# Kamino666/video_features

Measured on AMD Instinct MI355X. Metric: frames/sec CLIP-ViT-B/32 uni_12, higher is better.
Workload: dtype bf16; 1 GPU; model=CLIP-ViT-B/32, global_batch=256, seq_len=12, resolution=224, parallelism=dp1

## Files before the change

### video_features_amd/models/clip_vit.py

```python
from __future__ import annotations

from dataclasses import dataclass
from typing import Optional

import torch
import torch.nn.functional as F
from torch import nn

from .. import ops


@dataclass
class ViTConfig:
    input_resolution: int = 224
    patch_size: int = 32
    width: int = 768
    layers: int = 12
    heads: int = 12
    output_dim: int = 512


VIT_B32 = ViTConfig(patch_size=32)
VIT_B16 = ViTConfig(patch_size=16)


class LayerNorm(nn.LayerNorm):
    def forward(self, x: torch.Tensor) -> torch.Tensor:
        return ops.layer_norm(x, self.weight, self.bias, self.eps)


class MultiheadSelfAttention(nn.Module):
    def __init__(self, width: int, heads: int):
        super().__init__()
        self.heads = heads
        self.head_dim = width // heads
        self.qkv = nn.Linear(width, 3 * width)
        self.proj = nn.Linear(width, width)

    def forward(self, x: torch.Tensor) -> torch.Tensor:
        o = ops.mhsa_fused(self.qkv(x), self.heads)
        return self.proj(o)


class MLP(nn.Module):
    def __init__(self, width: int):
        super().__init__()
        self.c_fc = nn.Linear(width, 4 * width)
        self.c_proj = nn.Linear(4 * width, width)

    def forward(self, x: torch.Tensor) -> torch.Tensor:
        h = ops.linear_act(x, self.c_fc.weight, self.c_fc.bias, 'quick_gelu')
        return self.c_proj(h)


class ResidualAttentionBlock(nn.Module):
    def __init__(self, width: int, heads: int):
        super().__init__()
        self.ln_1 = LayerNorm(width)
        self.attn = MultiheadSelfAttention(width, heads)
        self.ln_2 = LayerNorm(width)
        self.mlp = MLP(width)

    def forward(self, x: torch.Tensor) -> torch.Tensor:
        x = x + self.attn(self.ln_1(x))
        x = x + self.mlp(self.ln_2(x))
        return x


class VisionTransformer(nn.Module):
    def __init__(self, cfg: ViTConfig = VIT_B32):
        super().__init__()
        self.cfg = cfg
        w = cfg.width
        self.conv1 = nn.Conv2d(3, w, kernel_size=cfg.patch_size,
                               stride=cfg.patch_size, bias=False)
        n_patches = (cfg.input_resolution // cfg.patch_size) ** 2
        scale = w ** -0.5
        self.class_embedding = nn.Parameter(scale * torch.randn(w))
        self.positional_embedding = nn.Parameter(
            scale * torch.randn(n_patches + 1, w))
        self.ln_pre = LayerNorm(w)
        self.blocks = nn.ModuleList(
            [ResidualAttentionBlock(w, cfg.heads) for _ in range(cfg.layers)])
        self.ln_post = LayerNorm(w)
        self.proj = nn.Parameter(scale * torch.randn(w, cfg.output_dim))

    def _patch_embed(self, x: torch.Tensor) -> torch.Tensor:
        if x.is_cuda:
            t = x.shape[0]
            p = self.cfg.patch_size
            g = x.shape[-1] // p
            xp = x.reshape(t, 3, g, p, g, p).permute(0, 2, 4, 1, 3, 5)
            xp = xp.reshape(t, g * g, 3 * p * p)
            w = self.conv1.weight.reshape(self.cfg.width, -1)
            return xp @ w.t()
        x = self.conv1(x)
        return x.flatten(2).transpose(1, 2)

    def forward(self, x: torch.Tensor) -> torch.Tensor:
        x = self._patch_embed(x)
        x = ops.clip_embed_ln(x, self.class_embedding,
                              self.positional_embedding, self.ln_pre.weight,
                              self.ln_pre.bias, self.ln_pre.eps)
        full_tail = ops._env_flag('VFA_CLIP_FULL_TAIL')
        delta, res = None, x
        for blk in (self.blocks if full_tail else self.blocks[:-1]):
            if delta is None:
                y1, s1 = blk.ln_1(res), res
            else:
                y1, s1 = ops.layer_norm_residual(delta, res, blk.ln_1.weight,
                                                 blk.ln_1.bias, blk.ln_1.eps)
            a = blk.attn(y1)
            y2, s2 = ops.layer_norm_residual(a, s1, blk.ln_2.weight,
                                             blk.ln_2.bias, blk.ln_2.eps)
            delta, res = blk.mlp(y2), s2
        if full_tail:
            x = delta + res
            x = self.ln_post(x[:, 0, :])
        else:
            x = self._cls_tail(self.blocks[-1], delta, res)
        return x @ self.proj.to(x.dtype)

    def _cls_tail(self, blk: ResidualAttentionBlock,
                  delta: Optional[torch.Tensor],
                  res: torch.Tensor) -> torch.Tensor:
        w = self.cfg.width
        if delta is None:
            y1, s1 = blk.ln_1(res), res
        else:
            y1, s1 = ops.layer_norm_residual(delta, res, blk.ln_1.weight,
                                             blk.ln_1.bias, blk.ln_1.eps)
        qkv = blk.attn.qkv
        kv = F.linear(y1, qkv.weight[w:], qkv.bias[w:])
        q = F.linear(y1[:, 0], qkv.weight[:w], qkv.bias[:w])
        o = ops.attention_pool(q, kv, blk.attn.heads)
        a = blk.attn.proj(o)
        y2, s2 = ops.layer_norm_residual(a, s1[:, 0], blk.ln_2.weight,
                                         blk.ln_2.bias, blk.ln_2.eps)
        d = blk.mlp(y2)
        y, _ = ops.layer_norm_residual(d, s2, self.ln_post.weight,
                                       self.ln_post.bias, self.ln_post.eps)
        return y

    def encode_image(self, x: torch.Tensor) -> torch.Tensor:
        return self.forward(x)


def build_clip_vit(feature_type: str) -> VisionTransformer:
    if feature_type in ('CLIP-ViT-B/32', 'CLIP4CLIP-ViT-B-32'):
        return VisionTransformer(VIT_B32)
    if feature_type == 'CLIP-ViT-B/16':
        return VisionTransformer(VIT_B16)
    raise ValueError(f'unknown CLIP feature type {feature_type!r}')
```

### video_features_amd/ops/__init__.py

```python
from __future__ import annotations

import math
import os
from typing import Optional

import torch

_ext = None
_ext_err: Optional[str] = None


def _env_flag(name: str) -> bool:
    return os.environ.get(name, '').strip().lower() not in (
        '', '0', 'false', 'no', 'off')


def _load_extension():
    global _ext, _ext_err
    if _ext is not None or _ext_err is not None:
        return _ext
    try:
        from . import _vfa_hip
        _ext = _vfa_hip
    except ImportError as e:
# ... 345 lines not shown
            and kv.dtype == torch.bfloat16 and d == 64 and c == heads * 64):
        return _ext.attention_pool(q.contiguous(), kv.contiguous(),
                                   int(heads))
    qh = q.float().view(b, heads, 1, d)
    kh = kv[..., :c].float().reshape(b, l, heads, d).permute(0, 2, 1, 3)
    vh = kv[..., c:].float().reshape(b, l, heads, d).permute(0, 2, 1, 3)
    attn = (qh @ kh.transpose(-2, -1)) / math.sqrt(d)
    o = attn.softmax(dim=-1) @ vh
    return o.reshape(b, c).to(q.dtype)


_ACT_IDS = {'none': 0, 'relu': 1, 'quick_gelu': 2, 'gelu': 3,
            'leaky_relu': 4}


def _act_id(act: str) -> int:
    if act not in _ACT_IDS:
        raise ValueError(f'unknown activation {act!r}; expected one of '
                         f'{sorted(_ACT_IDS)}')
    return _ACT_IDS[act]


def _apply_act(y: torch.Tensor, act: str) -> torch.Tensor:
    _act_id(act)
    if act == 'relu':
        return torch.nn.functional.relu(y)
    if act == 'quick_gelu':
        return y * torch.sigmoid(1.702 * y)
    if act == 'gelu':
        return torch.nn.functional.gelu(y, approximate='tanh')
    if act == 'leaky_relu':
        return torch.nn.functional.leaky_relu(y, 0.1)
    return y


def linear_act(x: torch.Tensor, weight: torch.Tensor,
               bias: Optional[torch.Tensor] = None,
               act: str = 'none',
               res: Optional[torch.Tensor] = None) -> torch.Tensor:
    k = x.shape[-1]
    n = weight.shape[0]
    if (_use_hip(x) and x.dtype == torch.bfloat16
            and weight.dtype == torch.bfloat16 and k % 8 == 0 and n >= 16
            and not _env_flag('VFA_NO_LTGEMM')):
        x2 = x.reshape(-1, k).contiguous()
        r2 = res.reshape(-1, n).contiguous() if res is not None else None
        out = _ext.linear_act(x2, weight.contiguous(), bias, r2,
                              _act_id(act))
        return out.reshape(*x.shape[:-1], n)
    y = torch.nn.functional.linear(x, weight, bias)
    if res is not None:
        y = y + res.reshape(y.shape)
    return _apply_act(y, act)


def temporal_merge_fused(y: torch.Tensor, b: int, kt: int, st: int,
                         p0: int, relu: bool = False,
                         p1: Optional[int] = None) -> Optional[torch.Tensor]:
    if (_use_hip(y)
            and y.is_contiguous(memory_format=torch.channels_last)):
        return _ext.temporal_merge(y, b, kt, st, p0,
                                   p0 if p1 is None else p1, relu)
    return None


def conv1x1_act(x: torch.Tensor, weight: torch.Tensor,
                bias: Optional[torch.Tensor] = None, act: str = 'none',
                res: Optional[torch.Tensor] = None) -> torch.Tensor:
    b, cin, h, w = x.shape
    x2 = x.permute(0, 2, 3, 1).reshape(-1, cin)
    r2 = res.permute(0, 2, 3, 1).reshape(-1, weight.shape[0]) \
        if res is not None else None
    y = linear_act(x2, weight.reshape(weight.shape[0], cin), bias, act, r2)
    return y.reshape(b, h, w, weight.shape[0]).permute(0, 3, 1, 2)


def conv2d_act(x: torch.Tensor, weight: torch.Tensor,
               bias: Optional[torch.Tensor] = None,
               stride=1, padding=0, act: str = 'none',
               res: Optional[torch.Tensor] = None,
               out: Optional[torch.Tensor] = None,
               out_off: int = 0, dilation=1, in_off: int = 0,
               in_ch: Optional[int] = None) -> torch.Tensor:
    sh, sw = (stride, stride) if isinstance(stride, int) else stride
    dh, dw = (dilation, dilation) if isinstance(dilation, int) else dilation
    if in_ch is None:
        if in_off:
            raise ValueError('conv2d_act: in_off needs in_ch')
        cx = x.shape[1]
    else:
        cx = in_ch
    if isinstance(padding, int):
        pt = pb = pl = pr = padding
    elif len(padding) == 2:
        pt = pb = padding[0]
        pl = pr = padding[1]
    else:
        pt, pb, pl, pr = padding
    if (_use_hip(x) and x.dtype == torch.bfloat16
            and weight.dtype == torch.bfloat16
            and weight.shape[1] == (cx + 7) // 8 * 8
            and (in_ch is None or (in_ch % 8 == 0 and in_off % 8 == 0
                                   and x.shape[1] % 8 == 0))
            and x.is_contiguous(memory_format=torch.channels_last)
            and not _env_flag('VFA_NO_CONV')):
        if (weight.shape[2] == 1 and weight.shape[3] == 1
# ... 247 lines not shown
```

### video_features_amd/ops/csrc/bindings.cpp

```cpp
#include <torch/extension.h>
#include <c10/hip/HIPStream.h>
#include <mutex>
#include <unordered_map>
#include <hip/hip_runtime.h>
#include <hip/hip_bf16.h>

extern "C" {
void vfa_quick_gelu(const void*, void*, long long, int, hipStream_t);
void vfa_gelu_tanh(const void*, void*, long long, int, hipStream_t);
void vfa_layer_norm(const void*, const void*, const void*, void*, long long,
                    int, float, int, hipStream_t);
void vfa_bilinear_warp(const void*, const void*, void*, int, int, int, int,
                       int, hipStream_t);
void vfa_bilinear_warp_nhwc(const void*, const void*, void*, int, int, int,
                            int, long long, long long, long long, long long,
                            float, hipStream_t);
void vfa_pwc_correlation_nhwc(const void*, const void*, void*, int, int, int,
                              int, int, int, hipStream_t);
long long vfa_tconv_lds_bytes(int, int);
void vfa_tconv_pform(const void*, const void*, const void*, void*, void*, int,
                     int, int, int, int, int, int, hipStream_t);
void vfa_tconv_direct(const void*, const void*, const void*, void*, int, int,
                      int, int, long long, long long, long long, long long,
                      int, int, hipStream_t);
void vfa_grid_sample(const void*, const void*, void*, long long, int, int,
                     int, int, int, int, hipStream_t);
void vfa_corr_repack(const void*, void*, int, int, int, int, int,
                     hipStream_t);
void vfa_pwc_correlation(const void*, const void*, const void*, void*, int,
                         int, int, int, int, int, int, hipStream_t);
void vfa_mhsa_small(const void*, const void*, const void*, void*, int, int,
                    int, float, int, hipStream_t);
void vfa_flash_qkv(const void*, void*, int, int, int, float, hipStream_t);
void vfa_mfma_gemm16(const void*, const void*, void*, hipStream_t);
void vfa_layer_norm_residual(const void*, const void*, const void*,
                             const void*, void*, void*, long long, int,
                             float, int, hipStream_t);
void vfa_u8_chw_norm(const void*, void*, long long, int, int, const float*,
                     const float*, int, hipStream_t);
void vfa_corr_lookup(const void*, const void*, const void*, const void*,
                     const void*, void*, int, int, int, int, int, int, int,
                     int, int, long long, int, int, int, int, hipStream_t);
void vfa_convex_upsample(const void*, const void*, void*, int, int, int, int,
                         int, hipStream_t);
void vfa_gru_zr(const void*, const void*, void*, void*, int, int, int,
                long long, int, int, hipStream_t);
void vfa_gru_out(const void*, const void*, void*, int, int, int, long long,
                 int, int, hipStream_t);
void vfa_instance_norm2d(const void*, void*, int, int, int, float, int, int,
                         int, hipStream_t);
void vfa_maxpool3d_same(const void*, void*, long long, int, int, int, int,
                        int, int, int, int, int, int, int, int, int, int,
                        int, int, hipStream_t);
void vfa_maxpool2d_same(const void*, void*, long long, int, int, int, int,
                        int, int, int, int, int, int, int, int, int,
                        hipStream_t);
void vfa_linear_act(const void*, const void*, const void*, const void*,
                    void*, int, int, int, int, hipStream_t);
void vfa_temporal_merge(const void*, void*, int, int, int, int, int, int,
                        int, long long, int, int, hipStream_t);
void vfa_conv2d_nhwc(const void*, const void*, const void*, const void*,
                     const void*, void*, int, int, int, int, int, int, int,
                     int, int, int, int, int, int, int, int, int, int, int,
                     hipStream_t);
void vfa_conv2d_pick_tile(int, int, int*, int*);
void vfa_pad2d_nhwc(const void*, void*, int, int, int, int, int, int, int,
                    int, int, hipStream_t);
void vfa_avgpool2d_nhwc(const void*, void*, long long, int, int, int, int,
                        int, int, hipStream_t);
void vfa_attnpool_tokens(const void*, const void*, void*, long long, int, int,
                         hipStream_t);
void vfa_attention_pool_d64(const void*, const void*, void*, long long, int,
                            int, float, hipStream_t);
void vfa_clip_embed_ln(const void*, const void*, const void*, const void*,
                       const void*, void*, long long, int, int, float, int,
                       hipStream_t);
}

namespace {

int dtype_tag(const torch::Tensor& t) {
  switch (t.scalar_type()) {
    case torch::kFloat32: return 0;
    case torch::kBFloat16: return 1;
    case torch::kFloat16: return 2;
    default:
      TORCH_CHECK(false, "unsupported dtype ", t.scalar_type());
  }
}

hipStream_t current_stream() {
  return c10::hip::getCurrentHIPStream().stream();
}

torch::Tensor quick_gelu(torch::Tensor x) {
  TORCH_CHECK(x.is_cuda() && x.is_contiguous());
  auto out = torch::empty_like(x);
  vfa_quick_gelu(x.data_ptr(), out.data_ptr(), x.numel(), dtype_tag(x),
                 current_stream());
  return out;
}

torch::Tensor gelu_tanh(torch::Tensor x) {
  TORCH_CHECK(x.is_cuda() && x.is_contiguous());
  auto out = torch::empty_like(x);
  vfa_gelu_tanh(x.data_ptr(), out.data_ptr(), x.numel(), dtype_tag(x),
                current_stream());
  return out;
}
// ... 368 lines not shown
                             std::vector<int64_t> out_sz, bool nhwc) {
  TORCH_CHECK(x.is_cuda() && x.dim() == 4);
  if (nhwc) {
    TORCH_CHECK(cl_contig(x), "channels_last expected");
  } else {
    TORCH_CHECK(x.is_contiguous());
  }
  auto out = nhwc
      ? torch::empty({x.size(0), out_sz[0], out_sz[1], x.size(1)},
                     x.options()).permute({0, 3, 1, 2})
      : torch::empty({x.size(0), x.size(1), out_sz[0], out_sz[1]},
                     x.options());
  vfa_maxpool2d_same(x.data_ptr(), out.data_ptr(), x.size(0),
                     (int)x.size(1), (int)x.size(2), (int)x.size(3),
                     (int)out_sz[0], (int)out_sz[1], (int)kernel[0],
                     (int)kernel[1], (int)stride[0], (int)stride[1],
                     (int)pad_front[0], (int)pad_front[1], nhwc ? 1 : 0,
                     dtype_tag(x), current_stream());
  return out;
}

torch::Tensor linear_act(torch::Tensor x, torch::Tensor w,
                         c10::optional<torch::Tensor> bias,
                         c10::optional<torch::Tensor> res, int64_t act) {
  TORCH_CHECK(x.is_cuda() && x.dim() == 2 && x.is_contiguous());
  TORCH_CHECK(w.dim() == 2 && w.is_contiguous());
  TORCH_CHECK(x.scalar_type() == torch::kBFloat16 &&
              w.scalar_type() == torch::kBFloat16);
  const int m = (int)x.size(0), kk = (int)x.size(1), n = (int)w.size(0);
  TORCH_CHECK(w.size(1) == kk && kk % 8 == 0, "K%8==0 required");
  TORCH_CHECK(act >= 0 && act <= 4, "linear_act: unknown activation id ",
              act);
  const void* bptr = nullptr;
  torch::Tensor bc;
  if (bias.has_value()) {
    bc = bias->contiguous().to(torch::kBFloat16);
    TORCH_CHECK(bc.numel() == n);
    bptr = bc.data_ptr();
  }
  const void* rptr = nullptr;
  if (res.has_value()) {
    TORCH_CHECK(res->is_contiguous() &&
                res->scalar_type() == torch::kBFloat16 &&
                res->numel() == (long long)m * n,
                "residual must be (M, N) bf16 contiguous");
    rptr = res->data_ptr();
  }
  auto out = torch::empty({m, n}, x.options());
  vfa_linear_act(x.data_ptr(), w.data_ptr(), bptr, rptr, out.data_ptr(), m,
                 n, kk, (int)act, current_stream());
  return out;
}

torch::Tensor conv2d_nhwc(torch::Tensor x, torch::Tensor w,
                          c10::optional<torch::Tensor> bias,
                          c10::optional<torch::Tensor> res,
                          int64_t stride_h, int64_t stride_w,
                          int64_t pt, int64_t pb, int64_t pl, int64_t pr,
                          int64_t act,
                          c10::optional<torch::Tensor> out_buf,
                          int64_t out_off, int64_t dil_h, int64_t dil_w,
                          int64_t in_off, int64_t in_ch) {
  TORCH_CHECK(x.is_cuda() && x.dim() == 4 && cl_contig(x),
              "x must be channels_last");
  TORCH_CHECK(w.dim() == 4 && cl_contig(w), "w must be channels_last");
  TORCH_CHECK(x.scalar_type() == torch::kBFloat16 &&
              w.scalar_type() == torch::kBFloat16);
  const bool slice = in_ch > 0;
  const int xc = (int)x.size(1);
  if (slice) {
    TORCH_CHECK(in_off >= 0 && in_off % 8 == 0 && in_ch % 8 == 0 &&
                xc % 8 == 0 && in_off + in_ch <= xc,
                "slice input needs in_off, in_ch and the buffer width to be "
                "multiples of 8 and the slice inside the buffer");
  } else {
    TORCH_CHECK(in_off == 0 && in_ch == 0, "in_off needs in_ch > 0");
  }
  TORCH_CHECK(dil_h >= 1 && dil_w >= 1 && stride_h >= 1 && stride_w >= 1);
  const int b = (int)x.size(0), c = slice ? (int)in_ch : xc;
  const int h = (int)x.size(2), ww = (int)x.size(3);
  const int kout = (int)w.size(0), kh = (int)w.size(2), kw = (int)w.size(3);
  const int c8 = (c + 7) / 8 * 8;
  TORCH_CHECK(w.size(1) == c8, "weight C must be input C padded up to 8");
  const int hp = h + (int)(pt + pb), wp = ww + (int)(pl + pr);
  const int ekh = (int)dil_h * (kh - 1) + 1, ekw = (int)dil_w * (kw - 1) + 1;
  TORCH_CHECK(hp >= ekh && wp >= ekw, "dilated filter larger than the input");
  const int oh = (hp - ekh) / (int)stride_h + 1;
  const int ow = (wp - ekw) / (int)stride_w + 1;
  auto stream = current_stream();
  const bool inline_pad = (c8 == c);
  torch::Tensor xp = x;
  if (!inline_pad && (pt > 0 || pb > 0 || pl > 0 || pr > 0 || c8 != c)) {
    xp = torch::empty({b, hp, wp, c8}, x.options());
    vfa_pad2d_nhwc(x.data_ptr(), xp.data_ptr(), b, h, ww, c, c8, (int)pt,
                   (int)pb, (int)pl, (int)pr, stream);
    xp = xp.permute({0, 3, 1, 2});
  }
  static std::unordered_map<int, torch::Tensor> zpages;
  static std::mutex zp_mu;
  torch::Tensor zpage;
  {
    std::lock_guard<std::mutex> lk(zp_mu);
    auto it = zpages.find((int)x.get_device());
    if (it == zpages.end()) {
      zpage = torch::zeros({512}, x.options());
      zpages.emplace((int)x.get_device(), zpage);
// ... 198 lines not shown
  TORCH_CHECK(pos.is_cuda() && pos.dim() == 2 && pos.is_contiguous());
  TORCH_CHECK(x.scalar_type() == torch::kBFloat16 &&
              pos.scalar_type() == torch::kBFloat16, "attnpool_tokens: bf16");
  const int64_t hw = x.size(1), c = x.size(2);
  TORCH_CHECK(hw >= 1 && c % 8 == 0, "attnpool_tokens: C % 8 == 0 required");
  TORCH_CHECK(pos.size(0) == hw + 1 && pos.size(1) == c,
              "positional embedding must be (HW+1, C)");
  auto t = torch::empty({x.size(0), hw + 1, c}, x.options());
  vfa_attnpool_tokens(x.data_ptr(), pos.data_ptr(), t.data_ptr(), x.size(0),
                      (int)hw, (int)c, current_stream());
  return t;
}

torch::Tensor attention_pool(torch::Tensor q, torch::Tensor kv,
                             int64_t heads) {
  TORCH_CHECK(q.is_cuda() && q.dim() == 2 && q.is_contiguous());
  TORCH_CHECK(kv.is_cuda() && kv.dim() == 3 && kv.is_contiguous());
  TORCH_CHECK(q.scalar_type() == torch::kBFloat16 &&
              kv.scalar_type() == torch::kBFloat16, "attention_pool: bf16");
  const int64_t b = q.size(0), c = q.size(1), l = kv.size(1);
  TORCH_CHECK(heads >= 1 && c == heads * 64,
              "attention_pool covers head_dim 64");
  TORCH_CHECK(kv.size(0) == b && kv.size(2) == 2 * c && l >= 1,
              "kv must be (B, L>=1, 2C)");
  auto out = torch::empty({b, c}, q.options());
  vfa_attention_pool_d64(q.data_ptr(), kv.data_ptr(), out.data_ptr(), b,
                         (int)heads, (int)l, 0.125f, current_stream());
  return out;
}

}

PYBIND11_MODULE(TORCH_EXTENSION_NAME, m) {
  m.def("quick_gelu", &quick_gelu);
  m.def("gelu_tanh", &gelu_tanh);
  m.def("layer_norm", &layer_norm);
  m.def("bilinear_warp", &bilinear_warp);
  m.def("grid_sample_bilinear", &grid_sample_bilinear);
  m.def("pwc_correlation", &pwc_correlation);
  m.def("mhsa", &mhsa);
  m.def("flash_qkv", &flash_qkv);
  m.def("mfma_gemm16", &mfma_gemm16);
  m.def("layer_norm_residual", &layer_norm_residual);
  m.def("clip_embed_ln", &clip_embed_ln);
  m.def("u8_chw_norm", &u8_chw_norm);
  m.def("corr_lookup", &corr_lookup);
  m.def("convex_upsample", &convex_upsample);
  m.def("gru_zr", &gru_zr);
  m.def("gru_out", &gru_out);
  m.def("instance_norm2d", &instance_norm2d);
  m.def("maxpool3d_same", &maxpool3d_same);
  m.def("maxpool2d_same", &maxpool2d_same);
  m.def("linear_act", &linear_act);
  m.def("conv2d_nhwc", &conv2d_nhwc);
  m.def("conv2d_tile", &conv2d_tile);
  m.def("conv_transpose2d_nhwc", &conv_transpose2d_nhwc);
  m.def("conv_transpose2d_small", &conv_transpose2d_small);
  m.def("bilinear_warp_nhwc", &bilinear_warp_nhwc);
  m.def("pwc_correlation_nhwc", &pwc_correlation_nhwc);
  m.def("temporal_merge", &temporal_merge);
  m.def("avgpool2d_nhwc", &avgpool2d_nhwc);
  m.def("attnpool_tokens", &attnpool_tokens);
  m.def("attention_pool", &attention_pool);
  m.attr("gfx_arch") = "gfx950";
}
```

### video_features_amd/ops/csrc/gemm.hip

```cpp
#include "mfma_tile.h"
#include <cstdlib>

namespace {

template <int ACT, bool HAS_RES>
__device__ __forceinline__ void epilogue_strips(
    const f32x4 (&acc)[8][4], float* ep, const __bf16* __restrict__ bias,
    const __bf16* __restrict__ res, __bf16* __restrict__ c, int n,
    long long row0, int col0, int lane) {
  const int lo = lane & 15, hi4 = lane >> 4;
  const int ec = (lane & 7) * 8;
  const int col = col0 + ec;
  float bf[8];
#pragma unroll
  for (int e = 0; e < 8; ++e) bf[e] = 0.f;
  if (bias) {
    const bf16x8 b8 = *reinterpret_cast<const bf16x8*>(bias + col);
#pragma unroll
    for (int e = 0; e < 8; ++e) bf[e] = (float)b8[e];
  }
#pragma unroll
  for (int mi = 0; mi < 8; ++mi) {
#pragma unroll
    for (int jj = 0; jj < 4; ++jj)
#pragma unroll
      for (int r = 0; r < 4; ++r)
        ep[(hi4 * 4 + r) * 64 + (((jj ^ hi4) << 4) | lo)] = acc[mi][jj][r];
    __builtin_amdgcn_s_waitcnt(0xc07f);
#pragma unroll
    for (int p = 0; p < 2; ++p) {
      const int er = p * 8 + (lane >> 3);
      const float* src = ep + er * 64 + (ec ^ (((er >> 2) & 3) << 4));
      const f32x4 v0 = *reinterpret_cast<const f32x4*>(src);
      const f32x4 v1 = *reinterpret_cast<const f32x4*>(src + 4);
      const long long o = (row0 + mi * 16 + er) * n + col;
      bf16x8 rr8{};
      if (HAS_RES) rr8 = *reinterpret_cast<const bf16x8*>(res + o);
      bf16x8 o8;
#pragma unroll
      for (int e = 0; e < 8; ++e) {
        float v = (e < 4 ? v0[e & 3] : v1[e & 3]) + bf[e];
        if (HAS_RES) v += (float)rr8[e];
        o8[e] = (__bf16)act_f(v, ACT);
      }
      *reinterpret_cast<bf16x8*>(c + o) = o8;
    }
    __builtin_amdgcn_s_waitcnt(0xc07f);
  }
}

template <int ACT, bool FULL, bool BIG>
__global__ __launch_bounds__(BIG ? 512 : 256)
void linear_act_kernel(const __bf16* __restrict__ a,
                       const __bf16* __restrict__ w,
                       const __bf16* __restrict__ bias,
                       const __bf16* __restrict__ res,
                       __bf16* __restrict__ c, int m, int n, int k,
                       int tiles_m, int tile_base) {
  constexpr int BM = BIG ? 256 : 128, BN = BIG ? 256 : 128;
  constexpr int WAVES = BIG ? 8 : 4;
  constexpr int WN = BIG ? 4 : 2;
  constexpr int MI = BIG ? 8 : 4;
  constexpr int NJ = 4;
  constexpr int TILE_A = BM * BK * 2, TILE_BB = BN * BK * 2;
  constexpr int THREADS = BIG ? 512 : 256;

  extern __shared__ __attribute__((aligned(1024))) char smem[];
  auto sA = [&](int buf) { return smem + buf * (TILE_A + TILE_BB); };
  auto sB = [&](int buf) {
    return smem + buf * (TILE_A + TILE_BB) + TILE_A;
  };

  const int wg = tile_base + xcd_remap(blockIdx.x, gridDim.x);
  const int tile_n = wg / tiles_m, tile_m = wg % tiles_m;
  const int m0 = tile_m * BM, n0 = tile_n * BN;

  const int lane = threadIdx.x & 63, wave = threadIdx.x >> 6;
  const int wm = wave / WN, wn = wave % WN;

  const int nk = (k + BK - 1) / BK;
  const int valid_m = m - m0, valid_n = n - n0;
  const bool tile_full = valid_m >= BM && valid_n >= BN;

  auto stage = [&](int buf, int kt) {
    const long long ko = (long long)kt * BK;
    if (tile_full && (FULL || kt + 1 < nk)) {
      stage_glds<BM, WAVES>(a + (long long)m0 * k + ko, k, sA(buf), wave,
                            lane);
      stage_glds<BN, WAVES>(w + (long long)n0 * k + ko, k, sB(buf), wave,
                            lane);
    } else {
      const int vk = (int)min((long long)BK, (long long)k - ko);
      stage_guard<BM, THREADS>(a + (long long)m0 * k + ko, k, valid_m, vk,
                               sA(buf), threadIdx.x);
      stage_guard<BN, THREADS>(w + (long long)n0 * k + ko, k, valid_n, vk,
                               sB(buf), threadIdx.x);
    }
  };

  stage(0, 0);

  f32x4 acc[MI][NJ];
#pragma unroll
  for (int i = 0; i < MI; ++i)
#pragma unroll
    for (int j = 0; j < NJ; ++j) acc[i][j] = f32x4{0.f, 0.f, 0.f, 0.f};

  for (int kt = 0; kt < nk; ++kt) {
    __syncthreads();
    const int cur = kt & 1;
    const long long ko_nxt = (long long)(kt + 1) * BK;
    const bool glds_nxt =
        (kt + 1 < nk) && tile_full && (FULL || kt + 2 < nk);
    if ((kt + 1 < nk) && !glds_nxt) stage(1 - cur, kt + 1);
#pragma unroll
    for (int kk = 0; kk < 2; ++kk) {
      mfma_kstep<MI, NJ>(sA(cur), sB(cur), wm * (MI * 16), wn * (NJ * 16),
                         kk, lane, acc, [&] {
        if (glds_nxt) {
          stage_glds_piece<BM, WAVES>(a + (long long)m0 * k + ko_nxt, k,
                                      sA(1 - cur), wave, lane, kk, 2);
          stage_glds_piece<BN, WAVES>(w + (long long)n0 * k + ko_nxt, k,
                                      sB(1 - cur), wave, lane, kk, 2);
        }
      });
    }
  }

  epilogue_frag_hoisted<ACT, MI, NJ, !BIG>(
      tile_full, acc, bias, res, c, m, n, n, m0 + wm * (MI * 16),
      n0 + wn * (NJ * 16), lane);
}

template <int ACT>
__global__ __launch_bounds__(512, 1)
void linear256p_kernel(const __bf16* __restrict__ a,
                       const __bf16* __restrict__ w,
                       const __bf16* __restrict__ bias,
                       const __bf16* __restrict__ res,
                       __bf16* __restrict__ c, int n, int k, int tiles_m,
                       int ntiles) {
  constexpr int TILE = 256 * BK * 2;
  extern __shared__ __attribute__((aligned(1024))) char smem_p[];
  auto sA = [&](int buf) { return smem_p + buf * (2 * TILE); };
  auto sB = [&](int buf) { return smem_p + buf * (2 * TILE) + TILE; };

  const int lane = threadIdx.x & 63, wave = threadIdx.x >> 6;
  const int wm = wave >> 2, wn = wave & 3;
  float* ep = reinterpret_cast<float*>(smem_p + 4 * TILE) + wave * (16 * 64);

  const int nk = k / BK;
  int v = blockIdx.x;
  int wg = xcd_remap(v, ntiles);
  int m0 = (wg % tiles_m) * 256, n0 = (wg / tiles_m) * 256;
  const __bf16* ap = a + (long long)m0 * k;
  const __bf16* wp = w + (long long)n0 * k;

  stage_glds<256, 8>(ap, k, sA(0), wave, lane);
  stage_glds<256, 8>(wp, k, sB(0), wave, lane);

  int it = 0;
  for (;;) {
    const int vn = v + gridDim.x;
    const bool more = vn < ntiles;
    int m0n = m0, n0n = n0;
    if (more) {
      const int wgn = xcd_remap(vn, ntiles);
      m0n = (wgn % tiles_m) * 256;
      n0n = (wgn / tiles_m) * 256;
    }
    const __bf16* apn = a + (long long)m0n * k;
    const __bf16* wpn = w + (long long)n0n * k;

    f32x4 acc[8][4];
#pragma unroll
    for (int i = 0; i < 8; ++i)
#pragma unroll
      for (int j = 0; j < 4; ++j) acc[i][j] = f32x4{0.f, 0.f, 0.f, 0.f};

    for (int kt = 0; kt < nk; ++kt, ++it) {
      __syncthreads();
      const int cur = it & 1;
      const bool last = kt + 1 == nk;
      const __bf16* an = last ? apn : ap + (long long)(kt + 1) * BK;
      const __bf16* wn_ = last ? wpn : wp + (long long)(kt + 1) * BK;
      const bool issue = !last || more;
#pragma unroll
      for (int kk = 0; kk < 2; ++kk) {
        mfma_kstep<8, 4>(sA(cur), sB(cur), wm * 128, wn * 64, kk, lane, acc,
                         [&] {
          if (issue) {
            stage_glds_piece<256, 8>(an, k, sA(1 - cur), wave, lane, kk, 2);
            stage_glds_piece<256, 8>(wn_, k, sB(1 - cur), wave, lane, kk, 2);
          }
        });
      }
    }

    const long long row0 = m0 + wm * 128;
    const int col0 = n0 + wn * 64;
    if (res)
      epilogue_strips<ACT, true>(acc, ep, bias, res, c, n, row0, col0, lane);
    else
      epilogue_strips<ACT, false>(acc, ep, bias, res, c, n, row0, col0,
                                  lane);
    if (!more) break;
    v = vn; m0 = m0n; n0 = n0n; ap = apn; wp = wpn;
  }
}

template <int ACT>
__global__ __launch_bounds__(512, 1)
void linear8p_kernel(const __bf16* __restrict__ a,
                     const __bf16* __restrict__ w,
                     const __bf16* __restrict__ bias,
                     const __bf16* __restrict__ res,
                     __bf16* __restrict__ c, int m, int n, int k,
                     int tiles_m, int tiles_n) {
  extern __shared__ __attribute__((aligned(1024))) char smem8[];
  const int nk = k >> 6;

  const int wg = xcd_remap(blockIdx.x, tiles_m * tiles_n);
  const int tile_n = wg / tiles_m, tile_m = wg % tiles_m;
  const int m0 = tile_m * 256, n0 = tile_n * 256;

  const int lane = threadIdx.x & 63, wave = threadIdx.x >> 6;
  const int lo = lane & 15, hi4 = lane >> 4;
  const int wm = wave >> 2, wn = wave & 3;

  auto LA = [&](int t, int q) { return smem8 + (t * 4 + q) * 8192; };
  auto LB = [&](int t, int h) {
    return smem8 + 65536 + (t * 4 + h) * 8192;
  };

  const int off = (wave * 1024 + lane * 16);
  const int off_log = swz(off);
  const int rib = off_log >> 7;
  const int kfrac = (off_log & 127) >> 1;

  const int a_row_off = rib < 32 ? rib : 96 + rib;
  auto stage_a = [&](int T, int q) {
    const int kt = T < nk ? T : 0;
    const __bf16* src =
        a + (long long)(m0 + q * 32 + a_row_off) * k + kt * 64 + kfrac;
    __builtin_amdgcn_global_load_lds(
        reinterpret_cast<const unsigned int*>(src),
        reinterpret_cast<unsigned int*>(LA(T & 1, q) + wave * 1024), 16, 0,
        0);
  };
  auto stage_b = [&](int T, int h) {
    const int kt = T < nk ? T : 0;
    const __bf16* src =
        w + (long long)(n0 + h * 64 + rib) * k + kt * 64 + kfrac;
    __builtin_amdgcn_global_load_lds(
        reinterpret_cast<const unsigned int*>(src),
        reinterpret_cast<unsigned int*>(LB(T % 3, h) + wave * 1024), 16, 0,
        0);
  };
// ... 191 lines not shown
            }
            *reinterpret_cast<bf16x8*>(c + row * n + col) = o8;
          } else {
            for (int e = 0; e < 8 && ec + e < jcols && col + e < n; ++e) {
              float v = (float)v8[e];
              if (bias) v += (float)bias[col + e];
              if (res) v += (float)res[row * n + col + e];
              c[row * n + col + e] = (__bf16)act_f(v, ACT);
            }
          }
        }
        if (mi == 0) __builtin_amdgcn_s_waitcnt(0xc07f);
      }
    }
  }
}

template <int ACT, int KF>
void launch_thin_kf(const void* a, const void* w, const void* bias,
                    const void* res, void* c, int m, int n, int nch, int k,
                    int m_blocks, size_t lds, hipStream_t stream) {
  hipLaunchKernelGGL((linear_thin_kernel<ACT, KF>),
                     dim3(m_blocks, (n + nch - 1) / nch), dim3(256), lds,
                     stream, (const __bf16*)a, (const __bf16*)w,
                     (const __bf16*)bias, (const __bf16*)res, (__bf16*)c,
                     m, n, nch, k);
}

template <int ACT>
bool launch_thin(const void* a, const void* w, const void* bias,
                 const void* res, void* c, int m, int n, int k,
                 hipStream_t stream) {
  if (k > 256 || k % 8 != 0 || k < 64 || m < 65536 || n % 8 != 0)
    return false;
  const int kc = (k + 31) / 32 * 32;
  const int nch_cap = 36352 / (kc + 8) / 16 * 16;
  const int nch = min((n + 15) & ~15, nch_cap);
  if (nch < 16) return false;
  const int m_blocks = (int)min(((long long)m + 127) / 128, 4096LL);
  const size_t lds = (size_t)nch * (kc + 8) * 2 + 4 * 16 * 72 * 2;
  switch (kc / 32) {
    case 2: launch_thin_kf<ACT, 2>(a, w, bias, res, c, m, n, nch, k, m_blocks, lds, stream); break;
    case 3: launch_thin_kf<ACT, 3>(a, w, bias, res, c, m, n, nch, k, m_blocks, lds, stream); break;
    case 4: launch_thin_kf<ACT, 4>(a, w, bias, res, c, m, n, nch, k, m_blocks, lds, stream); break;
    case 5: launch_thin_kf<ACT, 5>(a, w, bias, res, c, m, n, nch, k, m_blocks, lds, stream); break;
    case 6: launch_thin_kf<ACT, 6>(a, w, bias, res, c, m, n, nch, k, m_blocks, lds, stream); break;
    case 7: launch_thin_kf<ACT, 7>(a, w, bias, res, c, m, n, nch, k, m_blocks, lds, stream); break;
    case 8: launch_thin_kf<ACT, 8>(a, w, bias, res, c, m, n, nch, k, m_blocks, lds, stream); break;
    default: return false;
  }
  return true;
}

template <int ACT, bool BIG>
void launch_tile(const void* a, const void* w, const void* bias,
                 const void* res, void* c, int m, int n, int k,
                 hipStream_t stream) {
  constexpr int BM = BIG ? 256 : 128, BN = BIG ? 256 : 128;
  const int tiles_m = (m + BM - 1) / BM, tiles_n = (n + BN - 1) / BN;
  const size_t lds = 2 * (size_t)(BM + BN) * BK * 2;
  const bool full = (k % BK == 0);
  int tile_base = 0;
  if (BIG && full && m % 256 == 0 && n >= 256 && n % 8 == 0) {
    static const int ncu = [] {
      int dev = 0, v = 0;
      (void)hipGetDevice(&dev);
      (void)hipDeviceGetAttribute(&v, hipDeviceAttributeMultiprocessorCount,
                                  dev);
      return v > 0 ? v : 256;
    }();
    constexpr size_t lds_p = 160 * 1024;
    static bool attr_set = false;
    if (!attr_set) {
      (void)hipFuncSetAttribute(
          reinterpret_cast<const void*>(&linear256p_kernel<ACT>),
          hipFuncAttributeMaxDynamicSharedMemorySize, (int)lds_p);
      attr_set = true;
    }
    const int ntiles = tiles_m * (n / 256);
    hipLaunchKernelGGL((linear256p_kernel<ACT>),
                       dim3((unsigned)min(ntiles, ncu)), dim3(512), lds_p,
                       stream, (const __bf16*)a, (const __bf16*)w,
                       (const __bf16*)bias, (const __bf16*)res, (__bf16*)c,
                       n, k, tiles_m, ntiles);
    if (n % 256 == 0) return;
    tile_base = ntiles;
  }
  const dim3 grid(tiles_m * tiles_n - tile_base);
  if (full)
    hipLaunchKernelGGL((linear_act_kernel<ACT, true, BIG>), grid,
                       dim3(BIG ? 512 : 256), lds, stream, (const __bf16*)a,
                       (const __bf16*)w, (const __bf16*)bias,
                       (const __bf16*)res, (__bf16*)c, m, n, k, tiles_m,
                       tile_base);
  else
    hipLaunchKernelGGL((linear_act_kernel<ACT, false, BIG>), grid,
                       dim3(BIG ? 512 : 256), lds, stream, (const __bf16*)a,
                       (const __bf16*)w, (const __bf16*)bias,
                       (const __bf16*)res, (__bf16*)c, m, n, k, tiles_m,
                       tile_base);
}

template <int ACT>
void launch_linear(const void* a, const void* w, const void* bias,
                   const void* res, void* c, int m, int n, int k,
                   hipStream_t stream) {
  static const int env8p = getenv("VFA_8P") ? 1
                           : getenv("VFA_NO_8P") ? -1 : 0;
  if (launch_thin<ACT>(a, w, bias, res, c, m, n, k, stream)) return;
  const long long tiles = (long long)((m + 255) / 256) * ((n + 255) / 256);
  const bool big = n >= 256 && m % 256 == 0 && tiles >= 150;
  const bool want8p = env8p > 0 || (env8p == 0 && ACT == 0 && !big);
  if (want8p && launch_8p<ACT>(a, w, bias, res, c, m, n, k, stream)) return;
  if (big)
    launch_tile<ACT, true>(a, w, bias, res, c, m, n, k, stream);
  else
    launch_tile<ACT, false>(a, w, bias, res, c, m, n, k, stream);
}

}

extern "C" {

void vfa_linear_act(const void* a, const void* w, const void* bias,
                    const void* res, void* c, int m, int n, int k, int act,
                    hipStream_t stream) {
  dispatch_act(act, [&](auto id) {
    launch_linear<decltype(id)::value>(a, w, bias, res, c, m, n, k, stream);
  });
}

}
```

Before: 82690 frames/sec.

## Fold LayerNorm-2 into the MLP fc GEMM using row stats from the proj epilogue

The attention proj GEMM epilogue now adds the residual and also writes per-row partial mean/M2 statistics. The following c_fc GEMM runs on the un-normalized residual with LN-scaled weights, then applies the mean/rstd correction in its epilogue via precomputed column sums and a folded bias. This removes the standalone layer_norm_residual pass and its read/write of the activations between the two GEMMs. In exchange it adds stats traffic, a heavier epilogue, and cached folded weights, with possible precision loss from bf16-rounded folded weights and the correction step.

```diff
diff --git a/video_features_amd/models/clip_vit.py b/video_features_amd/models/clip_vit.py
--- a/video_features_amd/models/clip_vit.py
+++ b/video_features_amd/models/clip_vit.py
@@ -37,9 +37,11 @@
         self.qkv = nn.Linear(width, 3 * width)
         self.proj = nn.Linear(width, width)
 
+    def heads_out(self, x: torch.Tensor) -> torch.Tensor:
+        return ops.mhsa_fused(self.qkv(x), self.heads)
+
     def forward(self, x: torch.Tensor) -> torch.Tensor:
-        o = ops.mhsa_fused(self.qkv(x), self.heads)
-        return self.proj(o)
+        return self.proj(self.heads_out(x))
 
 
 class MLP(nn.Module):
@@ -60,11 +62,38 @@
         self.attn = MultiheadSelfAttention(width, heads)
         self.ln_2 = LayerNorm(width)
         self.mlp = MLP(width)
+        self._fold = None
 
     def forward(self, x: torch.Tensor) -> torch.Tensor:
         x = x + self.attn(self.ln_1(x))
         x = x + self.mlp(self.ln_2(x))
         return x
+
+    def _ln2_fold(self):
+        src = (self.mlp.c_fc.weight, self.mlp.c_fc.bias, self.ln_2.weight,
+               self.ln_2.bias)
+        key = tuple((p._version, p.data_ptr(), p.dtype, p.device)
+                    for p in src)
+        if self._fold is None or self._fold[0] != key:
+            with torch.no_grad():
+                self._fold = (key, ops.fold_ln_linear(*src))
+        return self._fold[1]
+
+    def fold_routed(self, x: torch.Tensor) -> bool:
+        if ops._env_flag('VFA_NO_LNFOLD'):
+            return False
+        return not x.is_cuda or (
+            ops.fused_ln_tiles(x, self.attn.proj.weight)
+            and ops.fused_ln_tiles(x, self.mlp.c_fc.weight))
+
+    def attn_mlp_folded(self, y1: torch.Tensor, s1: torch.Tensor):
+        proj, fc, ln = self.attn.proj, self.mlp.c_fc, self.ln_2
+        s2, st2 = ops.linear_res_stats(self.attn.heads_out(y1), proj.weight,
+                                       proj.bias, s1)
+        h = ops.linear_ln_act(
+            s2, st2, *self._ln2_fold(), act='quick_gelu', eps=ln.eps,
+            unfolded=(fc.weight, fc.bias, ln.weight, ln.bias))
+        return self.mlp.c_proj(h), s2
 
 
 class VisionTransformer(nn.Module):
@@ -110,6 +139,9 @@
             else:
                 y1, s1 = ops.layer_norm_residual(delta, res, blk.ln_1.weight,
                                                  blk.ln_1.bias, blk.ln_1.eps)
+            if blk.fold_routed(s1):
+                delta, res = blk.attn_mlp_folded(y1, s1)
+                continue
             a = blk.attn(y1)
             y2, s2 = ops.layer_norm_residual(a, s1, blk.ln_2.weight,
                                              blk.ln_2.bias, blk.ln_2.eps)
diff --git a/video_features_amd/ops/__init__.py b/video_features_amd/ops/__init__.py
--- a/video_features_amd/ops/__init__.py
+++ b/video_features_amd/ops/__init__.py
@@ -421,6 +421,68 @@
     if res is not None:
         y = y + res.reshape(y.shape)
     return _apply_act(y, act)
+
+
+def fused_ln_tiles(x: torch.Tensor, weight: torch.Tensor) -> bool:
+    k, n = x.shape[-1], weight.shape[0]
+    m = x.numel() // max(k, 1)
+    return bool(x.is_cuda and x.dtype == torch.bfloat16
+                and weight.dtype == torch.bfloat16
+                and m > 0 and m % 256 == 0 and n % 256 == 0 and k % 64 == 0
+                and not _env_flag('VFA_NO_LTGEMM') and _use_hip(x))
+
+
+def linear_res_stats(x: torch.Tensor, weight: torch.Tensor,
+                     bias: Optional[torch.Tensor], res: torch.Tensor):
+    n = weight.shape[0]
+    if fused_ln_tiles(x, weight):
+        s, stats = _ext.linear_res_stats(
+            x.reshape(-1, x.shape[-1]).contiguous(), weight.contiguous(),
+            bias, res.reshape(-1, n).contiguous())
+        return s.reshape(*x.shape[:-1], n), stats
+    s = linear_act(x, weight, bias, 'none', res)
+    sf = s.reshape(-1, n).float()
+    var, mean = torch.var_mean(sf, dim=1, unbiased=False)
+    return s, torch.stack([mean, var * n], dim=1).unsqueeze(1)
+
+
+def ln_stats(stats: torch.Tensor, n: int, eps: float = 1e-5) -> torch.Tensor:
+    gmean, gm2 = stats[..., 0], stats[..., 1]
+    mean = gmean.mean(dim=1, keepdim=True)
+    m2 = (gm2 + (n / stats.shape[1]) * (gmean - mean) ** 2).sum(dim=1)
+    return torch.stack([mean[:, 0], torch.rsqrt(m2 / n + eps)], dim=1)
+
+
+def fold_ln_linear(weight: torch.Tensor, bias: Optional[torch.Tensor],
+                   ln_weight: torch.Tensor, ln_bias: torch.Tensor):
+    acc = torch.float64 if weight.dtype == torch.float64 else torch.float32
+    w32 = weight.detach().to(acc)
+    wf = (w32 * ln_weight.detach().to(acc)).to(weight.dtype)
+    c = wf.double().sum(dim=1).to(acc)
+    bf = w32 @ ln_bias.detach().to(acc)
+    if bias is not None:
+        bf = bf + bias.detach().to(acc)
+    return wf.contiguous(), c.contiguous(), bf.contiguous()
+
+
+def linear_ln_act(s: torch.Tensor, stats: torch.Tensor, wf: torch.Tensor,
+                  c: torch.Tensor, bf: torch.Tensor, act: str = 'none',
+                  eps: float = 1e-5, unfolded=None) -> torch.Tensor:
+    n, k = wf.shape
+    if fused_ln_tiles(s, wf):
+        out = _ext.linear_ln_act(s.reshape(-1, k).contiguous(),
+                                 stats.contiguous(), wf.contiguous(), c, bf,
+                                 eps, _act_id(act))
+        return out.reshape(*s.shape[:-1], n)
+    if unfolded is not None:
+        weight, bias, ln_weight, ln_bias = unfolded
+        return linear_act(layer_norm(s, ln_weight, ln_bias, eps), weight,
+                          bias, act)
+    acc = torch.float64 if s.dtype == torch.float64 else torch.float32
+    st = ln_stats(stats.to(acc), k, eps)
+    y = s.reshape(-1, k).to(acc) @ wf.to(acc).t()
+    y = st[:, 1:2] * (y - st[:, 0:1] * c.to(acc)) + bf.to(acc)
+    return _apply_act(y, act).to(s.dtype).reshape(*s.shape[:-1], n)
 
 
 def temporal_merge_fused(y: torch.Tensor, b: int, kt: int, st: int,
diff --git a/video_features_amd/ops/csrc/bindings.cpp b/video_features_amd/ops/csrc/bindings.cpp
--- a/video_features_amd/ops/csrc/bindings.cpp
+++ b/video_features_amd/ops/csrc/bindings.cpp
@@ -55,6 +55,11 @@
 void vfa_maxpool2d_same(const void*, void*, long long, int, int, int, int,
                         int, int, int, int, int, int, int, int, int,
                         hipStream_t);
+void vfa_linear_res_stats(const void*, const void*, const void*, const void*,
+                          void*, void*, int, int, int, hipStream_t);
+void vfa_linear_ln_act(const void*, const void*, int, const void*,
+                       const void*, const void*, void*, int, int, int, float,
+                       int, hipStream_t);
 void vfa_linear_act(const void*, const void*, const void*, const void*,
                     void*, int, int, int, int, hipStream_t);
 void vfa_temporal_merge(const void*, void*, int, int, int, int, int, int,
@@ -529,6 +534,71 @@
   return out;
 }
 
+static void check_full_tiles(const char* op, int m, int n, int k) {
+  TORCH_CHECK(m > 0 && m % 256 == 0 && n % 256 == 0 && k % 64 == 0, op,
+              ": needs M % 256 == 0, N % 256 == 0, K % 64 == 0, got M=", m,
+              " N=", n, " K=", k);
+}
+
+std::vector<torch::Tensor> linear_res_stats(torch::Tensor x, torch::Tensor w,
+                                            c10::optional<torch::Tensor> bias,
+                                            torch::Tensor res) {
+  TORCH_CHECK(x.is_cuda() && x.dim() == 2 && x.is_contiguous());
+  TORCH_CHECK(w.dim() == 2 && w.is_contiguous());
+  TORCH_CHECK(x.scalar_type() == torch::kBFloat16 &&
+              w.scalar_type() == torch::kBFloat16);
+  const int m = (int)x.size(0), kk = (int)x.size(1), n = (int)w.size(0);
+  TORCH_CHECK(w.size(1) == kk);
+  check_full_tiles("linear_res_stats", m, n, kk);
+  const void* bptr = nullptr;
+  torch::Tensor bc;
+  if (bias.has_value()) {
+    bc = bias->contiguous().to(torch::kBFloat16);
+    TORCH_CHECK(bc.numel() == n);
+    bptr = bc.data_ptr();
+  }
+  TORCH_CHECK(res.is_cuda() && res.is_contiguous() &&
+              res.scalar_type() == torch::kBFloat16 &&
+              res.numel() == (long long)m * n,
+              "residual must be (M, N) bf16 contiguous");
+  auto out = torch::empty({m, n}, x.options());
+  auto stats = torch::empty({m, n / 256, 2},
+                            x.options().dtype(torch::kFloat32));
+  vfa_linear_res_stats(x.data_ptr(), w.data_ptr(), bptr, res.data_ptr(),
+                       out.data_ptr(), stats.data_ptr(), m, n, kk,
+                       current_stream());
+  return {out, stats};
+}
+
+torch::Tensor linear_ln_act(torch::Tensor x, torch::Tensor stats,
+                            torch::Tensor w, torch::Tensor ln_c,
+                            torch::Tensor ln_b, double eps, int64_t act) {
+  TORCH_CHECK(x.is_cuda() && x.dim() == 2 && x.is_contiguous());
+  TORCH_CHECK(w.is_cuda() && w.dim() == 2 && w.is_contiguous());
+  TORCH_CHECK(x.scalar_type() == torch::kBFloat16 &&
+              w.scalar_type() == torch::kBFloat16);
+  const int m = (int)x.size(0), kk = (int)x.size(1), n = (int)w.size(0);
+  TORCH_CHECK(w.size(1) == kk);
+  check_full_tiles("linear_ln_act", m, n, kk);
+  TORCH_CHECK(act >= 0 && act <= 4, "linear_ln_act: unknown activation id ",
+              act);
+  TORCH_CHECK(stats.is_cuda() && stats.is_contiguous() &&
+              stats.scalar_type() == torch::kFloat32 && stats.dim() == 3 &&
+              stats.size(0) == m && stats.size(2) == 2 &&
+              stats.size(1) >= 1 && kk % stats.size(1) == 0,
+              "stats must be (M, T, 2) f32 with K % T == 0");
+  for (const auto* v : {&ln_c, &ln_b})
+    TORCH_CHECK(v->is_cuda() && v->is_contiguous() &&
+                v->scalar_type() == torch::kFloat32 && v->numel() == n,
+                "ln_c / ln_b must be (N) f32");
+  auto out = torch::empty({m, n}, x.options());
+  vfa_linear_ln_act(x.data_ptr(), stats.data_ptr(), (int)stats.size(1),
+                    w.data_ptr(), ln_c.data_ptr(), ln_b.data_ptr(),
+                    out.data_ptr(), m, n, kk, (float)eps, (int)act,
+                    current_stream());
+  return out;
+}
+
 torch::Tensor conv2d_nhwc(torch::Tensor x, torch::Tensor w,
                           c10::optional<torch::Tensor> bias,
                           c10::optional<torch::Tensor> res,
@@ -833,6 +903,8 @@
   m.def("maxpool3d_same", &maxpool3d_same);
   m.def("maxpool2d_same", &maxpool2d_same);
   m.def("linear_act", &linear_act);
+  m.def("linear_res_stats", &linear_res_stats);
+  m.def("linear_ln_act", &linear_ln_act);
   m.def("conv2d_nhwc", &conv2d_nhwc);
   m.def("conv2d_tile", &conv2d_tile);
   m.def("conv_transpose2d_nhwc", &conv_transpose2d_nhwc);
diff --git a/video_features_amd/ops/csrc/gemm.hip b/video_features_amd/ops/csrc/gemm.hip
--- a/video_features_amd/ops/csrc/gemm.hip
+++ b/video_features_amd/ops/csrc/gemm.hip
@@ -3,18 +3,91 @@
 
 namespace {
 
-template <int ACT, bool HAS_RES>
+enum { EPI_PLAIN = 0, EPI_STATS = 1, EPI_LN = 2 };
+
+struct EpiExtra {
+  const float* ln_c;
+  const float* ln_b;
+  const float2* stats;
+  float2* part;
+  int groups;
+  float eps;
+};
+
+__device__ __forceinline__ float sum8(float v) {
+  auto dpp = [](float x, auto ctrl) {
+    return __builtin_bit_cast(
+        float, __builtin_amdgcn_update_dpp(0, __builtin_bit_cast(int, x),
+                                           decltype(ctrl)::value, 0xf, 0xf,
+                                           true));
+  };
+  v += dpp(v, std::integral_constant<int, 0xb1>{});
+  v += dpp(v, std::integral_constant<int, 0x4e>{});
+  v += dpp(v, std::integral_constant<int, 0x141>{});
+  return v;
+}
+
+__device__ __forceinline__ float bcast8(float v, int j, int l7) {
+  const int i = __builtin_bit_cast(int, v);
+  int b;
+  switch (j & 3) {
+    case 0: b = __builtin_amdgcn_update_dpp(0, i, 0x00, 0xf, 0xf, true); break;
+    case 1: b = __builtin_amdgcn_update_dpp(0, i, 0x55, 0xf, 0xf, true); break;
+    case 2: b = __builtin_amdgcn_update_dpp(0, i, 0xaa, 0xf, 0xf, true); break;
+    default: b = __builtin_amdgcn_update_dpp(0, i, 0xff, 0xf, 0xf, true);
+  }
+  const int m = __builtin_amdgcn_update_dpp(0, b, 0x141, 0xf, 0xf, true);
+  return __builtin_bit_cast(float, (l7 >> 2) == (j >> 2) ? b : m);
+}
+
+template <int ACT, bool HAS_RES, int MODE = EPI_PLAIN>
 __device__ __forceinline__ void epilogue_strips(
     const f32x4 (&acc)[8][4], float* ep, const __bf16* __restrict__ bias,
     const __bf16* __restrict__ res, __bf16* __restrict__ c, int n,
-    long long row0, int col0, int lane) {
+    long long row0, int col0, int lane, const EpiExtra& x = EpiExtra{},
+    int kdim = 0) {
   const int lo = lane & 15, hi4 = lane >> 4;
   const int ec = (lane & 7) * 8;
   const int col = col0 + ec;
-  float bf[8];
-#pragma unroll
-  for (int e = 0; e < 8; ++e) bf[e] = 0.f;
-  if (bias) {
+  float bf[8], cf[8];
+#pragma unroll
+  for (int e = 0; e < 8; ++e) bf[e] = cf[e] = 0.f;
+  const float gi = MODE == EPI_LN ? 1.f / (float)x.groups : 0.f;
+  const float gw = MODE == EPI_LN ? (float)(kdim / x.groups) : 0.f;
+  const int l7 = lane & 7;
+  float2 sp[2] = {float2{0.f, 0.f}, float2{0.f, 0.f}};
+  float2 own[2] = {float2{0.f, 1.f}, float2{0.f, 1.f}};
+  if (MODE == EPI_LN) {
+#pragma unroll
+    for (int h = 0; h < 2; ++h) {
+      const long long r =
+          row0 + h * 64 + (l7 >> 1) * 16 + (l7 & 1) * 8 + (lane >> 3);
+      const float2* pp = x.stats + r * x.groups;
+      const float m0 = pp[0].x;
+      float q = pp[0].y, s1 = 0.f, s2 = 0.f;
+      for (int i = 1; i < x.groups; ++i) {
+        const float2 g = pp[i];
+        const float d = g.x - m0;
+        s1 += d;
+        s2 = fmaf(d, d, s2);
+        q += g.y;
+      }
+      const float m2 = fmaf(gw, s2 - s1 * s1 * gi, q);
+      own[h] = float2{fmaf(s1, gi, m0), rsqrtf(fmaf(m2, gi / gw, x.eps))};
+    }
+  }
+  if (MODE == EPI_LN) {
+#pragma unroll
+    for (int h = 0; h < 2; ++h) {
+      const f32x4 b4 = *reinterpret_cast<const f32x4*>(x.ln_b + col + h * 4);
+      const f32x4 c4 = *reinterpret_cast<const f32x4*>(x.ln_c + col + h * 4);
+#pragma unroll
+      for (int e = 0; e < 4; ++e) {
+        bf[h * 4 + e] = b4[e];
+        cf[h * 4 + e] = c4[e];
+      }
+    }
+  } else if (bias) {
     const bf16x8 b8 = *reinterpret_cast<const bf16x8*>(bias + col);
 #pragma unroll
     for (int e = 0; e < 8; ++e) bf[e] = (float)b8[e];
@@ -33,19 +106,49 @@
       const float* src = ep + er * 64 + (ec ^ (((er >> 2) & 3) << 4));
       const f32x4 v0 = *reinterpret_cast<const f32x4*>(src);
       const f32x4 v1 = *reinterpret_cast<const f32x4*>(src + 4);
-      const long long o = (row0 + mi * 16 + er) * n + col;
+      const long long row = row0 + mi * 16 + er;
+      const long long o = row * n + col;
       bf16x8 rr8{};
       if (HAS_RES) rr8 = *reinterpret_cast<const bf16x8*>(res + o);
+      float2 st{0.f, 1.f};
+      if (MODE == EPI_LN) {
+        st.x = bcast8(own[mi >> 2].x, (mi * 2 + p) & 7, l7);
+        st.y = bcast8(own[mi >> 2].y, (mi * 2 + p) & 7, l7);
+      }
       bf16x8 o8;
 #pragma unroll
       for (int e = 0; e < 8; ++e) {
-        float v = (e < 4 ? v0[e & 3] : v1[e & 3]) + bf[e];
+        float v = e < 4 ? v0[e & 3] : v1[e & 3];
+        if (MODE == EPI_LN)
+          v = fmaf(st.y, fmaf(-st.x, cf[e], v), bf[e]);
+        else
+          v += bf[e];
         if (HAS_RES) v += (float)rr8[e];
         o8[e] = (__bf16)act_f(v, ACT);
       }
       *reinterpret_cast<bf16x8*>(c + o) = o8;
+      if (MODE == EPI_STATS) {
+        float s = 0.f;
+#pragma unroll
+        for (int e = 0; e < 8; ++e) s += (float)o8[e];
+        const float mean = sum8(s) * (1.f / 64.f);
+        float q = 0.f;
+#pragma unroll
+        for (int e = 0; e < 8; ++e) {
+          const float d = (float)o8[e] - mean;
+          q = fmaf(d, d, q);
+        }
+        q = sum8(q);
+        if (((mi * 2 + p) & 7) == l7) sp[mi >> 2] = float2{mean, q};
+      }
     }
     __builtin_amdgcn_s_waitcnt(0xc07f);
+  }
+  if (MODE == EPI_STATS) {
+    float2* ep2 = reinterpret_cast<float2*>(ep) + (l7 >> 1) * 16 +
+                  (l7 & 1) * 8 + (lane >> 3);
+    ep2[0] = sp[0];
+    ep2[64] = sp[1];
   }
 }
 
@@ -132,14 +235,14 @@
       n0 + wn * (NJ * 16), lane);
 }
 
-template <int ACT>
+template <int ACT, int MODE = EPI_PLAIN>
 __global__ __launch_bounds__(512, 1)
 void linear256p_kernel(const __bf16* __restrict__ a,
                        const __bf16* __restrict__ w,
                        const __bf16* __restrict__ bias,
                        const __bf16* __restrict__ res,
                        __bf16* __restrict__ c, int n, int k, int tiles_m,
-                       int ntiles) {
+                       int ntiles, EpiExtra x) {
   constexpr int TILE = 256 * BK * 2;
   extern __shared__ __attribute__((aligned(1024))) char smem_p[];
   auto sA = [&](int buf) { return smem_p + buf * (2 * TILE); };
@@ -199,11 +302,36 @@
 
     const long long row0 = m0 + wm * 128;
     const int col0 = n0 + wn * 64;
-    if (res)
-      epilogue_strips<ACT, true>(acc, ep, bias, res, c, n, row0, col0, lane);
+    if (MODE == EPI_LN)
+      epilogue_strips<ACT, false, MODE>(acc, ep, nullptr, nullptr, c, n,
+                                        row0, col0, lane, x, k);
+    else if (res)
+      epilogue_strips<ACT, true, MODE>(acc, ep, bias, res, c, n, row0, col0,
+                                       lane, x);
     else
-      epilogue_strips<ACT, false>(acc, ep, bias, res, c, n, row0, col0,
-                                  lane);
+      epilogue_strips<ACT, false, MODE>(acc, ep, bias, res, c, n, row0,
+                                        col0, lane, x);
+    if (MODE == EPI_STATS) {
+      __builtin_amdgcn_s_waitcnt(0xc07f);
+      __builtin_amdgcn_s_barrier();
+      if (threadIdx.x < 256) {
+        const float2* b2 =
+            reinterpret_cast<const float2*>(smem_p + 4 * TILE) +
+            (threadIdx.x >> 7) * 4 * 512 + (threadIdx.x & 127);
+        float2 g[4];
+#pragma unroll
+        for (int i = 0; i < 4; ++i) g[i] = b2[i * 512];
+        const float mean = 0.25f * ((g[0].x + g[1].x) + (g[2].x + g[3].x));
+        float m2 = 0.f;
+#pragma unroll
+        for (int i = 0; i < 4; ++i) {
+          const float d = g[i].x - mean;
+          m2 += fmaf(64.f * d, d, g[i].y);
+        }
+        x.part[(long long)(m0 + (int)threadIdx.x) * (n >> 8) + (n0 >> 8)] =
+            float2{mean, m2};
+      }
+    }
     if (!more) break;
     v = vn; m0 = m0n; n0 = n0n; ap = apn; wp = wpn;
   }
@@ -501,6 +629,32 @@
   return true;
 }
 
+template <int ACT, int MODE>
+void launch_256p(const void* a, const void* w, const void* bias,
+                 const void* res, void* c, int n, int k, int tiles_m,
+                 int ntiles, const EpiExtra& x, hipStream_t stream) {
+  static const int ncu = [] {
+    int dev = 0, v = 0;
+    (void)hipGetDevice(&dev);
+    (void)hipDeviceGetAttribute(&v, hipDeviceAttributeMultiprocessorCount,
+                                dev);
+    return v > 0 ? v : 256;
+  }();
+  constexpr size_t lds_p = 160 * 1024;
+  static bool attr_set = false;
+  if (!attr_set) {
+    (void)hipFuncSetAttribute(
+        reinterpret_cast<const void*>(&linear256p_kernel<ACT, MODE>),
+        hipFuncAttributeMaxDynamicSharedMemorySize, (int)lds_p);
+    attr_set = true;
+  }
+  hipLaunchKernelGGL((linear256p_kernel<ACT, MODE>),
+                     dim3((unsigned)min(ntiles, ncu)), dim3(512), lds_p,
+                     stream, (const __bf16*)a, (const __bf16*)w,
+                     (const __bf16*)bias, (const __bf16*)res, (__bf16*)c, n,
+                     k, tiles_m, ntiles, x);
+}
+
 template <int ACT, bool BIG>
 void launch_tile(const void* a, const void* w, const void* bias,
                  const void* res, void* c, int m, int n, int k,
@@ -511,27 +665,9 @@
   const bool full = (k % BK == 0);
   int tile_base = 0;
   if (BIG && full && m % 256 == 0 && n >= 256 && n % 8 == 0) {
-    static const int ncu = [] {
-      int dev = 0, v = 0;
-      (void)hipGetDevice(&dev);
-      (void)hipDeviceGetAttribute(&v, hipDeviceAttributeMultiprocessorCount,
-                                  dev);
-      return v > 0 ? v : 256;
-    }();
-    constexpr size_t lds_p = 160 * 1024;
-    static bool attr_set = false;
-    if (!attr_set) {
-      (void)hipFuncSetAttribute(
-          reinterpret_cast<const void*>(&linear256p_kernel<ACT>),
-          hipFuncAttributeMaxDynamicSharedMemorySize, (int)lds_p);
-      attr_set = true;
-    }
     const int ntiles = tiles_m * (n / 256);
-    hipLaunchKernelGGL((linear256p_kernel<ACT>),
-                       dim3((unsigned)min(ntiles, ncu)), dim3(512), lds_p,
-                       stream, (const __bf16*)a, (const __bf16*)w,
-                       (const __bf16*)bias, (const __bf16*)res, (__bf16*)c,
-                       n, k, tiles_m, ntiles);
+    launch_256p<ACT, EPI_PLAIN>(a, w, bias, res, c, n, k, tiles_m, ntiles,
+                                EpiExtra{}, stream);
     if (n % 256 == 0) return;
     tile_base = ntiles;
   }
@@ -579,4 +715,30 @@
   });
 }
 
-}
+void vfa_linear_res_stats(const void* a, const void* w, const void* bias,
+                          const void* res, void* c, void* part, int m, int n,
+                          int k, hipStream_t stream) {
+  EpiExtra x{};
+  x.part = (float2*)part;
+  launch_256p<0, EPI_STATS>(a, w, bias, res, c, n, k, m / 256,
+                            (m / 256) * (n / 256), x, stream);
+}
+
+void vfa_linear_ln_act(const void* a, const void* stats, int groups,
+                       const void* w, const void* ln_c, const void* ln_b,
+                       void* c, int m, int n, int k, float eps, int act,
+                       hipStream_t stream) {
+  EpiExtra x{};
+  x.ln_c = (const float*)ln_c;
+  x.ln_b = (const float*)ln_b;
+  x.stats = (const float2*)stats;
+  x.groups = groups;
+  x.eps = eps;
+  dispatch_act(act, [&](auto id) {
+    launch_256p<decltype(id)::value, EPI_LN>(a, w, nullptr, nullptr, c, n, k,
+                                             m / 256, (m / 256) * (n / 256),
+                                             x, stream);
+  });
+}
+
+}
```

After: 84400 frames/sec (median of 6 runs). 1.02x the previous value.
